# jinseikenai/glomeruli_segmentation

Measured on AMD Instinct MI355X. Metric: patches/sec (1024x512 RGB) ESPNet p=2 q=8 5 classes, HBM-resident, two batches in flight, higher is better.
Workload: dtype f32; 1 GPU; ESPNet p=2 q=8 encoder+decoder, batch=32 synthetic 1024x512 uint8 BGR tiles per GPU, normalise+forward+argmax+counts, inputs resident in HBM, steps rotate through 4 distinct batches, 2 batch(es) in flight (engine lanes, one HIP stream each) for `value`; global_batch=32, weights=espnet_fold1 (tests/golden), parallelism=tile-range per rank x1

## Files before the change

### glomeruli_segmentation_amd/build.py

```python
import os
import subprocess
import sys
import tempfile

PKG = os.path.dirname(os.path.abspath(__file__))
CSRC = os.path.join(PKG, "csrc")
LIB = os.path.join(PKG, "libglomseg.so")
SOURCES = ["espnet.hip", "dec_tail.hip", "crops.hip", "detect_ops.hip", "detector.hip", "wsi_eval.hip", "contours.cpp"]
HEADERS = ["gs_internal.h", "conv_mfma.h", "dec_tail.h", "dec_tail_args.h", "espnet_kernels.h", "crop_sample.h", "crop_plan.h", "host_copy.h", "host_jobs.h", "host_pipe.h",
           os.path.join("..", "..", "include", "glomseg.h")]
FLAGS = ["-O3", "--offload-arch=gfx950", "-std=c++17", "-fPIC", "-Wall", "-Wno-unused-result",
         "-Wno-unused-value"]


def _sources():
    return [s for s in SOURCES if os.path.exists(os.path.join(CSRC, s))]


def _stale(lib):
    if not os.path.exists(lib):
        return True
    t = os.path.getmtime(lib)
    deps = [os.path.join(CSRC, s) for s in _sources() + HEADERS] + [os.path.abspath(__file__)]
    deps += [os.path.join(CSRC, f) for f in os.listdir(CSRC) if f.endswith(".h") or f.endswith(".inc")]
    return any(os.path.getmtime(d) > t for d in deps)


def build_lib(force=False, verbose=False, out=None, extra_flags=()):
    lib = os.path.abspath(out) if out else LIB
    if not (force or _stale(lib)):
        return lib
    hipcc = os.environ.get("HIPCC", "/opt/rocm/bin/hipcc")
    os.makedirs(os.path.dirname(lib), exist_ok=True)
    objdir = CSRC if out is None else tempfile.mkdtemp(prefix="glomseg_obj_")
    objs = []
    procs = []
    for s in _sources():
        o = os.path.join(objdir, s.replace(".hip", ".o").replace(".cpp", ".o"))
        objs.append(o)
        cmd = [hipcc] + FLAGS + list(extra_flags) + (["-x", "hip"] if s.endswith(".cpp") else []) + ["-c", os.path.join(CSRC, s), "-o", o]
        if verbose:
            print(" ".join(cmd))
        procs.append((cmd, subprocess.Popen(cmd)))
    for cmd, p in procs:
        if p.wait() != 0:
            raise RuntimeError("hipcc failed: " + " ".join(cmd))
    cmd = [hipcc, "--offload-arch=gfx950", "-shared", "-fPIC", "-o", lib] + objs + ["-Wl,-rpath,/opt/rocm/lib"]
    if verbose:
        print(" ".join(cmd))
    subprocess.check_call(cmd)
    return lib


if __name__ == "__main__":
    argv = sys.argv[1:]
    extra = []
    if "--" in argv:
        extra = argv[argv.index("--") + 1:]
        argv = argv[:argv.index("--")]
    out = argv[argv.index("--out") + 1] if "--out" in argv else None
    print(build_lib(force="--force" in argv or out is not None, verbose=True, out=out, extra_flags=extra))
```

### glomeruli_segmentation_amd/csrc/conv_mfma.h

```cpp
#pragma once
#include <map>
#include <mutex>
#include <type_traits>

#include "gs_internal.h"

namespace gs {

#ifdef GS_DIAG
constexpr bool kDiag = true;
#else
constexpr bool kDiag = false;
#endif

template <int N, typename F>
__device__ __forceinline__ void static_for(F &&f)
{
    if constexpr (N > 0) {
        static_for<N - 1>(f);
        f(std::integral_constant<int, N - 1>{});
    }
}

typedef float f32x16 __attribute__((ext_vector_type(16)));
typedef float f32x4 __attribute__((ext_vector_type(4)));

template <int MT>
struct Mfma;
template <>
struct Mfma<32> {
    static constexpr int KL = 2, NACC = 16;
    using acc_t = f32x16;
    static __device__ __forceinline__ acc_t run(float a, float b, acc_t c)
    {
        return __builtin_amdgcn_mfma_f32_32x32x2f32(a, b, c, 0, 0, 0);
    }
    static __device__ __forceinline__ int row(int r, int kq) { return (r & 3) + 8 * (r >> 2) + 4 * kq; }
};
template <>
struct Mfma<16> {
    static constexpr int KL = 4, NACC = 4;
    using acc_t = f32x4;
    static __device__ __forceinline__ acc_t run(float a, float b, acc_t c)
    {
        return __builtin_amdgcn_mfma_f32_16x16x4f32(a, b, c, 0, 0, 0);
    }
    static __device__ __forceinline__ int row(int r, int kq) { return kq * 4 + r; }
};

struct ConvArgs {
    const float *in;
    long long in_sn;
    int in_sc, in_pitch, in_off;
    unsigned in_img_bytes;
    const float *wpack;
    int wfloats;
    float *out;
    long long out_sn;
    int out_sc, out_pitch, out_off;
    unsigned out_img_bytes, res_img_bytes;
    const float *res;
    long long res_sn;
    int res_sc, res_pitch, res_off;
    float *out2;
    long long out2_sn;
    int out2_sc, out2_pitch, out2_off, out2_coff;
    unsigned out2_img_bytes;
    float *out3;
    long long out3_sn;
    int out3_sc, out3_pitch, out3_off, nout3;
    unsigned out3_img_bytes;
    int bnl_s0, bnl_s1;
    int stagger;
    int prio_mode;
    unsigned long long *stamp;
    int N, H, W;
    int strips;
    int total_tasks;
    int wu;
};

typedef unsigned u32x3_t __attribute__((ext_vector_type(3)));
typedef unsigned u32x2_t __attribute__((ext_vector_type(2)));
typedef unsigned u32x4_t __attribute__((ext_vector_type(4)));

template <int N, int AUX = 0>
__device__ __forceinline__ void buf_load_vec(const __amdgpu_buffer_rsrc_t &rs, int voff, int soff, float *dst)
{
    if constexpr (N == 1) {
        dst[0] = __builtin_bit_cast(float, __builtin_amdgcn_raw_buffer_load_b32(rs, voff, soff, AUX));
    } else if constexpr (N == 2) {
        const u32x2_t v = __builtin_amdgcn_raw_buffer_load_b64(rs, voff, soff, AUX);
        const unsigned e0 = v[0], e1 = v[1];
        dst[0] = __builtin_bit_cast(float, e0);
        dst[1] = __builtin_bit_cast(float, e1);
    } else {
        static_assert(N == 4 || N == 8, "vector width");
#pragma unroll
        for (int h = 0; h < N / 4; ++h) {
            const u32x4_t v = __builtin_amdgcn_raw_buffer_load_b128(rs, voff + 16 * h, soff, AUX);
            const unsigned e0 = v[0], e1 = v[1], e2 = v[2], e3 = v[3];
            dst[4 * h + 0] = __builtin_bit_cast(float, e0);
            dst[4 * h + 1] = __builtin_bit_cast(float, e1);
            dst[4 * h + 2] = __builtin_bit_cast(float, e2);
            dst[4 * h + 3] = __builtin_bit_cast(float, e3);
        }
    }
}
template <int N, int AUX = 0>
__device__ __forceinline__ void buf_store_vec(const __amdgpu_buffer_rsrc_t &rs, int voff, const float *src)
{
    if constexpr (N == 1) {
        __builtin_amdgcn_raw_buffer_store_b32(__builtin_bit_cast(unsigned, src[0]), rs, voff, 0, AUX);
    } else if constexpr (N == 2) {
        u32x2_t v;
        v[0] = __builtin_bit_cast(unsigned, src[0]);
        v[1] = __builtin_bit_cast(unsigned, src[1]);
        __builtin_amdgcn_raw_buffer_store_b64(v, rs, voff, 0, AUX);
    } else {
#pragma unroll
        for (int h = 0; h < N / 4; ++h) {
            u32x4_t v;
#pragma unroll
            for (int j = 0; j < 4; ++j)
                v[j] = __builtin_bit_cast(unsigned, src[4 * h + j]);
            __builtin_amdgcn_raw_buffer_store_b128(v, rs, voff + 16 * h, 0, AUX);
        }
    }
}

__device__ __forceinline__ float prelu_pin(float alpha)
{
    return alpha <= 1.0f ? __builtin_inff() : -__builtin_inff();
}
__device__ __forceinline__ float prelu_med3(float v, float alpha, float pin)
{
    return __builtin_amdgcn_fmed3f(v, alpha * v, pin);
}

constexpr int F_BNACT = 1;
constexpr int F_RES = 2;
constexpr int F_NOSTORE = 4;
constexpr int F_DUAL = 8;
constexpr int F_S2PAIR = 512;
constexpr int F_VEC = 1024;
constexpr int F_RES_NT = 8192;
constexpr int F_ST_NT = 16384;
constexpr int F_ST2_NT = 32768;
constexpr int F_IN_NT = 65536;
constexpr int F_A_GLOBAL = 131072;
constexpr int F_FUSE1X1 = 262144;
constexpr int F_S2_FLIP = 1048576;
constexpr int F_SKIP_PAD = 4194304;
constexpr int F_BNLOAD = 8388608;
constexpr int F_X_NOLOAD = 16;
constexpr int F_X_NOLDS = 32;
constexpr int F_X_NOEPI = 64;
constexpr int F_X_STAMP2 = 4096;
constexpr int STAMP2_SLOTS = 128;
constexpr int F_X_STAMP = 128;
constexpr int F_X_NOEPIMEM = 2097152;
constexpr int F_X_RESL2 = 33554432;
constexpr int F_X_STL2 = 67108864;
constexpr int F_X_ALL = F_X_NOLOAD | F_X_NOLDS | F_X_NOEPI | F_X_STAMP | F_X_STAMP2 | F_X_NOEPIMEM | F_X_RESL2 | F_X_STL2;

struct ConvImage {
    int nrow, cout, w, bn, tab, total;
};
constexpr ConvImage conv_image(int CINP, int TAPS, int NDIL, int NOUT1, int NOUT, bool bn, bool dual = false, int fuse_nacc = 0)
{
    ConvImage im{};
    im.nrow = NOUT1 > NOUT ? NOUT1 : NOUT;
    im.cout = NOUT1 + (NDIL - 1) * NOUT;
    im.w = NDIL * TAPS * CINP * im.nrow;
    im.bn = (bn ? 3 * im.cout : 0) + (dual ? 3 * im.cout : 0);
    im.tab = NDIL * fuse_nacc * 64;
    im.total = (im.w + im.bn + im.tab + 3) / 4 * 4;
    return im;
}

#ifndef CFG_STAGE_ROT
#define CFG_STAGE_ROT 17
#endif
#ifndef CFG_L3_RING
#define CFG_L3_RING 13
#endif
#ifndef CFG_L2_RING
#define CFG_L2_RING 27
#endif
constexpr int conv_ring_depth(int MT, int TAPS, int NDIL, int P, int G)
{
    return (MT == 32 && TAPS == 9 && NDIL == 5 && (P == 1 || P == 2) && G == 13) ? CFG_L3_RING
           : (MT == 16 && TAPS == 9 && NDIL == 5 && P == 4 && G == 9) ? CFG_L2_RING
                                                                    : G * (TAPS == 9 ? 3 : 1);
}

#define M_KL_OF(MT_) (Mfma<MT_>::KL)
template <int MT, int WAVES, int CINP, int TAPS, int STRIDE, int NDIL, int NOUT1, int NOUT, int P, int G, int FLAGS>
__global__ void __launch_bounds__(WAVES * 64, WAVES >= 8 ? WAVES / 8 : 2) conv_mfma_kernel(const ConvArgs a)
{
    constexpr bool BNACT = FLAGS & F_BNACT, RES = FLAGS & F_RES, STORE1 = !(FLAGS & F_NOSTORE), DUAL = FLAGS & F_DUAL;
    constexpr bool S2P = FLAGS & F_S2PAIR;
    constexpr bool VEC = FLAGS & F_VEC;
    constexpr bool AGL = FLAGS & F_A_GLOBAL, FUSE = FLAGS & F_FUSE1X1;
    constexpr bool S2FLIP = FLAGS & F_S2_FLIP;
    constexpr bool SKIP = FLAGS & F_SKIP_PAD;
    constexpr bool BNL = FLAGS & F_BNLOAD;
    static_assert(!BNL || ((FLAGS & F_S2PAIR) && !(FLAGS & (F_BNACT | F_A_GLOBAL | F_VEC))), "F_BNLOAD is for the plain stride-2 reduce");
    static_assert(!SKIP || (TAPS == 9 && STRIDE == 1 && !(FLAGS & F_S2PAIR) && G * M_KL_OF(MT) == CINP),
                  "F_SKIP_PAD: unit-stride 3x3 with one tap row per chunk");
    static_assert(!S2FLIP || (STRIDE == 2 && TAPS == 9 && NDIL == 1), "F_S2_FLIP is for the stride-2 3x3 reduce");
    static_assert(kDiag || !(FLAGS & F_X_ALL), "timing / stamp variants exist in -DGS_DIAG builds only");
    constexpr int IAUX = (FLAGS & F_IN_NT) ? 2 : 0;
    constexpr int RAUX = (FLAGS & F_RES_NT) ? 2 : 0, SAUX = (FLAGS & F_ST_NT) ? 2 : 0, SAUX2 = (FLAGS & F_ST2_NT) ? 2 : 0;
    static_assert(!VEC || (STRIDE == 1 && (P == 2 || P == 4 || P == 8)), "F_VEC needs unit stride and P in {2,4,8}");
    static_assert(!S2P || (STRIDE == 2 && TAPS == 9 && NDIL == 1), "F_S2PAIR is for the stride-2 3x3 reduce");
    using M = Mfma<MT>;
    constexpr int KL = M::KL;
    constexpr int NSTEP = CINP / KL;
    constexpr int NROW = NOUT1 > NOUT ? NOUT1 : NOUT;
    constexpr int COUT = NOUT1 + (NDIL - 1) * NOUT;
    constexpr int TYN = TAPS == 1 ? 1 : 3;
    constexpr int TXN = TAPS == 9 ? 3 : 1;
    constexpr int XSTEP = P * MT;
    constexpr int RGN = TYN * NSTEP;
    constexpr int D = G * TXN;
    constexpr int R = conv_ring_depth(MT, TAPS, NDIL, P, G);
    constexpr int RA = R;
    static_assert(D % R == 0 && (R == D || !(FLAGS & (F_S2PAIR | F_BNLOAD))), "the ring divides the chunk");
    constexpr int CPD = RGN / G;
    constexpr int NCHUNK = NDIL * CPD;
    static_assert(CINP % KL == 0, "k-steps must tile");
    static_assert(TAPS == 1 || TAPS == 9, "1x1 or 3x3");
    static_assert(RGN % G == 0, "chunk must divide the row groups of one dilation");
    static_assert(NROW <= MT, "one MFMA row block");
    constexpr int KSTR = 4;

    extern __shared__ __attribute__((aligned(16))) float lds[];
    const int tid = threadIdx.x;
    unsigned long long tstamp0 = 0;
    if (FLAGS & (F_X_STAMP | F_X_STAMP2))
        tstamp0 = __builtin_amdgcn_s_memrealtime();
    constexpr int WFL = NDIL * TAPS * CINP * NROW;
    constexpr int LDS_SRC0 = AGL ? WFL : 0;
    static_assert(!AGL || WFL % 4 == 0, "LDS-DMA source must stay 16-byte aligned");
    static_assert(!FUSE || (TAPS == 9 && BNACT), "the fused 1x1 follows a branch kernel's epilogue");
    const float *bnp = lds + (WFL - LDS_SRC0);
    constexpr int BNFL = (BNACT ? 3 * COUT : 0) + (DUAL ? 3 * COUT : 0);
    const float *tab = bnp + BNFL;
    constexpr int BNL_C = CINP + M::KL;
    const float *bnl = lds + (conv_image(CINP, TAPS, NDIL, NOUT1, NOUT, BNACT, DUAL, FUSE ? M::NACC : 0).total - LDS_SRC0);
    const __amdgpu_buffer_rsrc_t rsrc_w =
        __builtin_amdgcn_make_buffer_rsrc(const_cast<float *>(a.wpack), 0, AGL ? WFL * 4 : 0, 0x00020000);

    const int lane = tid & 63;
    const int wid = __builtin_amdgcn_readfirstlane(tid >> 6);
    const int px = lane % MT, kq = lane / MT;
    const int xl = VEC ? px * P : px;
    const int voff = (kq * a.in_sc + xl * STRIDE) * 4;
    const int lbase = kq * NROW + (px < NROW ? px : NROW - 1);
    const int vout = (kq * KSTR * a.out_sc + xl) * 4;
    const int vres = RES ? (kq * KSTR * a.res_sc + xl) * 4 : 0;
    const int vout2 = DUAL ? (kq * KSTR * a.out2_sc + xl) * 4 : 0;
    const int vout3 = FUSE ? (kq * KSTR * a.out3_sc + xl) * 4 : 0;
    const int prio_mode = kDiag ? a.prio_mode : 1;
    const bool second_of_simd = WAVES >= 8 ? wid >= WAVES / 2 : blockIdx.x >= gridDim.x / 2;

    const int NB = gridDim.x;
    const int wu = a.wu;
    int t0, t1, tstride;
    if ((NB & 7) == 0) {
        const int xcd = blockIdx.x & 7, per = NB >> 3;
        const int c0 = (int)((long long)a.total_tasks * xcd / 8), c1 = (int)((long long)a.total_tasks * (xcd + 1) / 8);
        t0 = c0 + (blockIdx.x >> 3) * wu + wid;
        t1 = c1;
        tstride = per * wu;
    } else {
        t0 = blockIdx.x * wu + wid;
        t1 = a.total_tasks;
        tstride = NB * wu;
    }
    if (wid >= wu)
        t0 = t1;
    const long long wg = (long long)blockIdx.x * WAVES + wid;
    const int tasks_per_img = a.H * a.strips;
    bool staged = false;

    float aq[RA], bq[S2P ? 1 : R][P];
    float bl[S2P ? G : 1][P][3];

    for (int task = t0; task < t1 || !staged; task += tstride) {
        const bool idle = task >= t1;
        const int tk = idle ? (a.total_tasks - 1) : task;
        const int n = tk / tasks_per_img;
        const int rem = tk - n * tasks_per_img;
        const int img_stride = tstride / tasks_per_img > 0 ? tstride / tasks_per_img : 1;
        const int yrot = SKIP ? a.H / 2 : 0;
        const int y0r = rem / a.strips;
        const int y = SKIP && ((n / img_stride) & 1) ? (y0r + yrot >= a.H ? y0r + yrot - a.H : y0r + yrot) : y0r;
        const int x0 = (rem - y0r * a.strips) * XSTEP;

        const __amdgpu_buffer_rsrc_t rsrc = __builtin_amdgcn_make_buffer_rsrc(
            const_cast<float *>(a.in + (long long)n * a.in_sn), 0, a.in_img_bytes, 0x00020000);
        const int sbase = (a.in_off + y * STRIDE * a.in_pitch + x0 * STRIDE) * 4;
        const int tn = task + tstride < t1 ? task + tstride : tk;
        const int n_n = tn / tasks_per_img;
        const int rem_n = tn - n_n * tasks_per_img;
        const int y0r_n = rem_n / a.strips;
        const int y_n = SKIP && ((n_n / img_stride) & 1) ? (y0r_n + yrot >= a.H ? y0r_n + yrot - a.H : y0r_n + yrot) : y0r_n;
        const __amdgpu_buffer_rsrc_t rsrc_n = __builtin_amdgcn_make_buffer_rsrc(
            const_cast<float *>(a.in + (long long)n_n * a.in_sn), 0, a.in_img_bytes, 0x00020000);
        const int sbase_n = (a.in_off + y_n * STRIDE * a.in_pitch + (rem_n - y0r_n * a.strips) * XSTEP * STRIDE) * 4;
        const bool flip = S2FLIP && (y & 1), flip_n = S2FLIP && (y_n & 1);
        const __amdgpu_buffer_rsrc_t rout =
            __builtin_amdgcn_make_buffer_rsrc(a.out + (long long)n * a.out_sn, 0, a.out_img_bytes, 0x00020000);
        const int sout = (a.out_off + y * a.out_pitch + x0) * 4;
        const __amdgpu_buffer_rsrc_t rres = __builtin_amdgcn_make_buffer_rsrc(
            const_cast<float *>(RES ? a.res + (long long)n * a.res_sn : a.in), 0, RES ? a.res_img_bytes : 0u, 0x00020000);
        const int sres = RES ? (a.res_off + y * a.res_pitch + x0) * 4 : 0;
        const __amdgpu_buffer_rsrc_t rout2 = __builtin_amdgcn_make_buffer_rsrc(
            DUAL ? a.out2 + (long long)n * a.out2_sn : a.out, 0, DUAL ? a.out2_img_bytes : 0u, 0x00020000);
        const int sout2 = DUAL ? (a.out2_off + y * a.out2_pitch + x0) * 4 : 0;
        const __amdgpu_buffer_rsrc_t rout3 = __builtin_amdgcn_make_buffer_rsrc(
            FUSE ? a.out3 + (long long)n * a.out3_sn : a.out, 0, FUSE ? a.out3_img_bytes : 0u, 0x00020000);
        const int sout3 = FUSE ? (a.out3_off + y * a.out3_pitch + x0) * 4 : 0;

        typename M::acc_t acc[P];
        typename M::acc_t acc2[FUSE ? P : 1];
        auto chunk_live = [&](int yy, int c) {
            const int di = c / CPD, ty = c - di * CPD;
            return ty == 1 || (ty == 0 ? yy >= (1 << di) : yy + (1 << di) < a.H);
        };
        const int c_first = SKIP && !chunk_live(y, 0) ? 1 : 0;
        const int c_first_n = SKIP && !chunk_live(y_n, 0) ? 1 : 0;

        constexpr int OOB = 0x7ffffff0;
        int vo[P], vr[P], vo2[P], vo3[P];
#pragma unroll
        for (int p = 0; p < P; ++p) {
            const bool xok = x0 + (VEC ? xl : p * MT + px) < a.W;
            vo[p] = xok ? vout + (VEC ? 0 : p * MT * 4) : OOB;
            vr[p] = xok ? vres + (VEC ? 0 : p * MT * 4) : OOB;
            vo2[p] = xok ? vout2 + (VEC ? 0 : p * MT * 4) : OOB;
            vo3[p] = xok ? vout3 + (VEC ? 0 : p * MT * 4) : OOB;
        }
        constexpr int RR = RES ? M::NACC : 1;
        float resv[RR][P];
        auto load_res = [&](int di, int r) {
            if (!RES)
                return;
            if (FLAGS & F_X_NOEPIMEM) {
#pragma unroll
                for (int p = 0; p < P; ++p)
                    resv[r % RR][p] = __builtin_bit_cast(float, di + r + p);
                return;
            }
            const int nout = di == 0 ? NOUT1 : NOUT;
            const int cb = di == 0 ? 0 : NOUT1 + (di - 1) * NOUT;
            const int ch0 = M::row(r, 0);
            const bool live = ch0 + kq * KSTR < nout;
            const int sr = (cb + ch0) * a.res_sc * 4 + sres;
            if (VEC) {
                if (FLAGS & F_X_RESL2)
                    buf_load_vec<P, RAUX>(rres, live ? ((int)(wg & 255) * 8192 + ((vr[0] + sr) & 0x1ff0)) : OOB, 0, resv[r % RR]);
                else
                    buf_load_vec<P, RAUX>(rres, live ? vr[0] : OOB, sr, resv[r % RR]);
                return;
            }
#pragma unroll
            for (int p = 0; p < P; ++p)
                resv[r % RR][p] = __builtin_bit_cast(
                    float, __builtin_amdgcn_raw_buffer_load_b32(rres, live ? vr[p] : OOB, sr, RAUX));
        };
        auto prefetch_res = [&](int di) {
#pragma unroll
            for (int r = 0; r < RR; ++r)
                load_res(di, r);
        };

        auto decode_rg = [&](int cw, int g, int &ty0, int &sidx) {
            if constexpr (G % NSTEP == 0) {
                ty0 = cw * (G / NSTEP) + g / NSTEP;
                sidx = g % NSTEP;
            } else if constexpr (NSTEP % G == 0) {
                constexpr int CPR = NSTEP / G;
                ty0 = cw / CPR;
                sidx = (cw - ty0 * CPR) * G + g;
            } else {
                const int rg = cw * G + g;
                ty0 = rg / NSTEP;
                sidx = rg - ty0 * NSTEP;
            }
        };
        auto fetch_b = [&](const __amdgpu_buffer_rsrc_t &rs, int sb, int c, int g, int tx, bool fl) {
            const int di = c / CPD;
            int ty0, sidx;
            decode_rg(c - di * CPD, g, ty0, sidx);
            const int ty = S2FLIP && fl ? TYN - 1 - ty0 : ty0;
            const int toff = TAPS == 9 ? ((ty - 1) * a.in_pitch + (tx - 1)) << di : 0;
            const int soff = sb + (toff + sidx * KL * a.in_sc) * 4;
            if ((FLAGS & F_X_NOLOAD) && staged)
                return;
            if (VEC) {
                buf_load_vec<P, IAUX>(rs, voff, soff, bq[S2P ? 0 : (g * TXN + tx) % R]);
                return;
            }
#pragma unroll
            for (int p = 0; p < P; ++p)
                bq[(g * TXN + tx) % R][p] = __builtin_bit_cast(
                    float, __builtin_amdgcn_raw_buffer_load_b32(rs, voff + p * MT * STRIDE * 4, soff, IAUX));
        };
        auto fetch_pair = [&](const __amdgpu_buffer_rsrc_t &rs, int sb, int c, int g, bool fl) {
            if ((FLAGS & F_X_NOLOAD) && staged)
                return;
            int ty0, sidx;
            decode_rg(c, g, ty0, sidx);
            const int ty = S2FLIP && fl ? TYN - 1 - ty0 : ty0;
            const int soff = sb + ((ty - 1) * a.in_pitch - 1 + sidx * KL * a.in_sc) * 4;
#pragma unroll
            for (int p = 0; p < P; ++p) {
                const u32x3_t v = __builtin_amdgcn_raw_buffer_load_b96(rs, voff + p * MT * STRIDE * 4, soff, IAUX);
                const unsigned e0 = v[0], e1 = v[1], e2 = v[2];
                bl[g][p][0] = __builtin_bit_cast(float, e0);
                bl[g][p][1] = __builtin_bit_cast(float, e1);
                bl[g][p][2] = __builtin_bit_cast(float, e2);
            }
        };
        auto fetch_a = [&](int c, int g, int tx, bool fl) {
            const int di = c / CPD;
            int ty0, sidx;
            decode_rg(c - di * CPD, g, ty0, sidx);
            const int ty = S2FLIP && fl ? TYN - 1 - ty0 : ty0;
            const int tap = TAPS == 9 ? ty * 3 + tx : 0;
            if ((FLAGS & F_X_NOLDS) && staged)
                return;
            if (AGL)
                aq[(g * TXN + tx) % R] = __builtin_bit_cast(
                    float, __builtin_amdgcn_raw_buffer_load_b32(rsrc_w, lbase * 4, (((di * TAPS + tap) * CINP + sidx * KL) * NROW) * 4, 0));
            else
                aq[(g * TXN + tx) % R] = lds[((di * TAPS + tap) * CINP + sidx * KL) * NROW + lbase];
        };

        auto bnl_fetch = [&](int cc, int gg, int yy, bool ff, float &sc2, float &sh2, float &al2, bool &raw) {
            int ty0c, sidxc;
            decode_rg(cc, gg, ty0c, sidxc);
            const int tyc = S2FLIP && ff ? TYN - 1 - ty0c : ty0c;
            raw = sidxc >= a.bnl_s0 && sidxc < a.bnl_s1;
            const bool padrow = yy * STRIDE + tyc - 1 < 0 && raw;
            const int ch = (padrow ? NSTEP : sidxc) * KL + kq;
            sc2 = bnl[ch];
            sh2 = bnl[BNL_C + ch];
            al2 = bnl[2 * BNL_C + ch];
        };
        float tsc = 1.0f, tsh = 0.0f, tal = 1.0f, tpin = 0.0f;
        float nsc = 1.0f, nsh = 0.0f, nal = 1.0f;
        bool traw = false, nraw = false;
        float bt[BNL ? 2 : 1][P][3];
        static_assert(!BNL || G % 2 == 0, "F_BNLOAD: the two-group operand buffer alternates by row-group parity");
        auto bnl_apply = [&](float &dst, float v, float sc2, float sh2, float al2, float pin2, bool zero) {
            v = v * sc2 + sh2;
            v = prelu_med3(v, al2, pin2);
            dst = zero ? 0.0f : v;
        };

        if (task == t0) {
#pragma unroll
            for (int g = 0; g < G; ++g) {
                if (S2P) {
                    fetch_pair(rsrc, sbase, 0, g, flip);
                    continue;
                }
#pragma unroll
                for (int tx = 0; tx < TXN; ++tx)
                    if (g * TXN + tx < R)
                        fetch_b(rsrc, sbase, c_first, g, tx, flip);
            }
        }
        if (!staged) {
            const int pieces = (a.wfloats - LDS_SRC0 + 255) / 256;
            if ((FLAGS & F_X_STAMP2) && lane == 0)
                a.stamp[wg * STAMP2_SLOTS + STAMP2_SLOTS - 2] = __builtin_amdgcn_s_memrealtime();
            const int rot = (int)((blockIdx.x * (unsigned)CFG_STAGE_ROT) % (unsigned)(pieces > 0 ? pieces : 1));
            for (int j0 = wid; j0 < pieces; j0 += WAVES) {
                const int j = j0 + rot < pieces ? j0 + rot : j0 + rot - pieces;
                __builtin_amdgcn_global_load_lds(
                    (const __attribute__((address_space(1))) void *)(a.wpack + LDS_SRC0 + j * 256 + lane * 4),
                    (__attribute__((address_space(3))) void *)(lds + j * 256), 16, 0, 0);
            }
            if ((FLAGS & F_X_STAMP2) && lane == 0)
                a.stamp[wg * STAMP2_SLOTS + STAMP2_SLOTS - 1] = __builtin_amdgcn_s_memrealtime();
            __syncthreads();
            staged = true;
        }
        if (idle)
            break;
        if ((FLAGS & F_X_STAMP) && lane == 0 && task == t0) {
            a.stamp[wg * 8 + 0] = tstamp0;
            a.stamp[wg * 8 + 1] = __builtin_amdgcn_s_memrealtime();
        }
        if ((FLAGS & F_X_STAMP2) && lane == 0 && task == t0) {
            a.stamp[wg * STAMP2_SLOTS + 0] = tstamp0;
            a.stamp[wg * STAMP2_SLOTS + 1] = __builtin_amdgcn_s_memrealtime();
        }
        const int ti_ = (FLAGS & F_X_STAMP2) ? (task - t0) / tstride : 0;
        const bool stamp2 = (FLAGS & F_X_STAMP2) && lane == 0 && 2 + (ti_ + 1) * 2 * NCHUNK <= STAMP2_SLOTS;
        const long long sbase2 = wg * STAMP2_SLOTS + 2 + ti_ * 2 * NCHUNK;
        if (kDiag && a.stagger > 0 && task == t0) {
            const int ph = second_of_simd ? 1 : 0;
            for (int z = 0; z < a.stagger * ph; ++z)
                __builtin_amdgcn_s_sleep(16);
        }
        if (task == t0) {
#pragma unroll
            for (int g = 0; g < G; ++g)
#pragma unroll
                for (int tx = 0; tx < TXN; ++tx)
                    if (g * TXN + tx < R)
                        fetch_a(c_first, g, tx, flip);
        }

        if (BNL) {
            bnl_fetch(c_first, 0, y, flip, tsc, tsh, tal, traw);
            bnl_fetch(c_first, 1, y, flip, nsc, nsh, nal, nraw);
            tpin = prelu_pin(tal);
#pragma unroll
            for (int p = 0; p < P; ++p)
#pragma unroll
                for (int t = 0; t < 3; ++t)
                    bnl_apply(bt[0][p][t], bl[0][p][t], tsc, tsh, tal, tpin, t == 0 && p == 0 && x0 == 0 && px == 0);
        }
        if (FUSE) {
#pragma unroll
            for (int p = 0; p < P; ++p)
                acc2[p] = (typename M::acc_t)(0.0f);
        }
        if (prio_mode == 1) {
            if ((((task - t0) / tstride) + (second_of_simd ? 1 : 0)) & 1)
                __builtin_amdgcn_s_setprio(1);
            else
                __builtin_amdgcn_s_setprio(0);
        } else if (prio_mode == 3 && task == t0) {
            if (second_of_simd)
                __builtin_amdgcn_s_setprio(1);
        }

        struct EpiParams {
            float scale = 1.0f, shift = 0.0f, alpha = 1.0f, scale2 = 1.0f, shift2 = 0.0f, alpha2 = 1.0f, a2 = 0.0f;
        };
        auto epi_params = [&](int di, auto r_) __attribute__((always_inline)) {
            constexpr int r = decltype(r_)::value;
            const int nout = di == 0 ? NOUT1 : NOUT;
            const int cb = di == 0 ? 0 : NOUT1 + (di - 1) * NOUT;
            const int ch0 = M::row(r, 0);
            const bool live = ch0 + kq * KSTR < nout;
            EpiParams q;
            q.a2 = (FUSE && BNACT) ? tab[(di * M::NACC + r) * 64 + lane] : 0.0f;
            if (BNACT) {
                const float *bp = bnp + (live ? cb + ch0 + kq * KSTR : 0);
                q.scale = bp[0];
                q.shift = bp[COUT];
                q.alpha = bp[2 * COUT];
                if (DUAL) {
                    q.scale2 = bp[3 * COUT];
                    q.shift2 = bp[4 * COUT];
                    q.alpha2 = bp[5 * COUT];
                }
            }
            return q;
        };
        auto epi_reg = [&](int di, auto r_) __attribute__((always_inline)) {
            constexpr int r = decltype(r_)::value;
            const int nout = di == 0 ? NOUT1 : NOUT;
            const int cb = di == 0 ? 0 : NOUT1 + (di - 1) * NOUT;
            const int ch0 = M::row(r, 0);
            const bool live = ch0 + kq * KSTR < nout;
            const EpiParams q = epi_params(di, r_);
            const float a2 = q.a2;
            const int so = (cb + ch0) * a.out_sc * 4 + sout;
            const int so2 = DUAL ? (a.out2_coff + cb + ch0) * a.out2_sc * 4 + sout2 : 0;
            const float scale = q.scale, shift = q.shift, alpha = q.alpha, scale2 = q.scale2, shift2 = q.shift2, alpha2 = q.alpha2;
            float o1[P], o2[P];
            const float pin = prelu_pin(alpha), pin2 = prelu_pin(alpha2);
#pragma unroll
            for (int p = 0; p < P; ++p) {
                float v = acc[p][r];
                if (RES)
                    v += resv[r % RR][p];
                if (BNACT) {
                    v = v * scale + shift;
                    v = prelu_med3(v, alpha, pin);
                }
                o1[p] = v;
                if (!VEC && STORE1)
                    __builtin_amdgcn_raw_buffer_store_b32(__builtin_bit_cast(unsigned, v), rout, live ? vo[p] : OOB, so, SAUX);
                if (DUAL) {
                    float v2 = v * scale2 + shift2;
                    v2 = prelu_med3(v2, alpha2, pin2);
                    o2[p] = v2;
                    if (!VEC)
                        __builtin_amdgcn_raw_buffer_store_b32(__builtin_bit_cast(unsigned, v2), rout2,
                                                              live ? vo2[p] : OOB, so2, SAUX2);
                }
            }
            if (VEC && STORE1 && !(FLAGS & F_X_NOEPIMEM))
                buf_store_vec<P, SAUX>(rout, live ? ((FLAGS & F_X_STL2) ? ((int)(wg & 255) * 8192 + ((vo[0] + so) & 0x1ff0)) : vo[0] + so) : OOB, o1);
            if (VEC && DUAL)
                buf_store_vec<P, SAUX2>(rout2, live ? vo2[0] + so2 : OOB, o2);
            if (FUSE && ch0 < nout) {
#pragma unroll
                for (int p = 0; p < P; ++p)
                    acc2[p] = M::run(a2, o1[p], acc2[p]);
            }
        };

        for (int c = 0; c < NCHUNK; ++c) {
            if (NDIL > 1 && c % CPD == 0 && prio_mode == 0) {
                if (((c / CPD) + (second_of_simd ? 1 : 0)) & 1)
                    __builtin_amdgcn_s_setprio(1);
                else
                    __builtin_amdgcn_s_setprio(0);
            }
            if (RES && c % CPD == 0)
                prefetch_res(c / CPD);
            if (c % CPD == 0 && c < 2 * CPD) {
#pragma unroll
                for (int p = 0; p < P; ++p)
                    acc[p] = (typename M::acc_t)(0.0f);
            }
            int nxl = c + 1;
            if (SKIP)
                while (nxl < NCHUNK && !chunk_live(y, nxl))
                    ++nxl;
            const bool last = nxl >= NCHUNK;
            const int nx = last ? c_first_n : nxl;
            const __amdgpu_buffer_rsrc_t rs = last ? rsrc_n : rsrc;
            const int sb = last ? sbase_n : sbase;
            const bool fl = last ? flip_n : flip;
            auto refill = [&](int u) __attribute__((always_inline)) {
                const int v = u + R;
                if (v < D && R < D) {
                    fetch_b(rsrc, sbase, c, v / TXN, v % TXN, flip);
                    fetch_a(c, v / TXN, v % TXN, flip);
                } else {
                    const int gn = (v - D) / TXN, txn = (v - D) % TXN;
                    if (!S2P)
                        fetch_b(rs, sb, nx, gn, txn, fl);
                    else if (txn == 2)
                        fetch_pair(rs, sb, nx, gn, fl);
                    fetch_a(nx, gn, txn, fl);
                }
            };
            if (!SKIP || chunk_live(y, c)) {
#pragma unroll
            for (int g = 0; g < G; ++g)
#pragma unroll
                for (int tx = 0; tx < TXN; ++tx) {
                    const int u = g * TXN + tx;
                    const bool ahead = BNL && (g + 1 < G || !last);
                    if (BNL && tx == 0) {
                        tsc = nsc;
                        tsh = nsh;
                        tal = nal;
                        traw = nraw;
                        tpin = prelu_pin(tal);
                        if (g + 2 < G)
                            bnl_fetch(c, g + 2, y, flip, nsc, nsh, nal, nraw);
                        else if (!last)
                            bnl_fetch(nx, g + 2 - G, y, flip, nsc, nsh, nal, nraw);
                    }
#pragma unroll
                    for (int p = 0; p < P; ++p) {
                        acc[p] = M::run(aq[u % RA], BNL ? bt[BNL ? g & 1 : 0][p][S2P ? tx : 0]
                                                       : S2P ? bl[S2P ? g : 0][p][S2P ? tx : 0] : bq[S2P ? 0 : u % R][p], acc[p]);
                        if (ahead) {
                            const int e = tx * P + p;
                            if (e < 3 * P)
                                bnl_apply(bt[BNL ? (g + 1) & 1 : 0][e / 3][e % 3], bl[S2P ? (g + 1) % G : 0][e / 3][e % 3], tsc, tsh, tal, tpin,
                                          e == 0 && x0 == 0 && px == 0);
                        }
                    }
                    refill(u);
                    __builtin_amdgcn_sched_barrier(0);
                }
            }
            if (stamp2)
                a.stamp[sbase2 + 2 * c] = __builtin_amdgcn_s_memrealtime();
            if ((c + 1) % CPD != 0)
                continue;
            if (FLAGS & F_X_NOEPI) {
                float keep = 0.0f;
#pragma unroll
                for (int p = 0; p < P; ++p)
#pragma unroll
                    for (int r = 0; r < M::NACC; ++r)
                        keep += acc[p][r];
                if (keep == 123.456f)
                    __builtin_amdgcn_raw_buffer_store_b32(__builtin_bit_cast(unsigned, keep), rout, vout, sout, 0);
                continue;
            }
            const int di = c / CPD;
            static_for<M::NACC>([&](auto r_) { epi_reg(di, r_); });
            if (FUSE && di + 1 == NDIL) {
#pragma unroll
                for (int r = 0; r < M::NACC; ++r) {
                    const int ch0 = M::row(r, 0);
                    if (ch0 >= a.nout3)
                        continue;
                    const bool live3 = ch0 + kq * KSTR < a.nout3;
                    const int so3 = ch0 * a.out3_sc * 4 + sout3;
                    float o3[P];
#pragma unroll
                    for (int p = 0; p < P; ++p) {
                        o3[p] = acc2[p][r];
                        if (!VEC)
                            __builtin_amdgcn_raw_buffer_store_b32(__builtin_bit_cast(unsigned, o3[p]), rout3, live3 ? vo3[p] : OOB, so3, 0);
                    }
                    if (VEC)
                        buf_store_vec<P, 0>(rout3, live3 ? vo3[0] + so3 : OOB, o3);
                }
            }
            if ((FLAGS & F_X_STAMP) && lane == 0 && task == t0)
                a.stamp[wg * 8 + 2 + di] = __builtin_amdgcn_s_memrealtime();
            if (stamp2)
                a.stamp[sbase2 + 2 * c + 1] = __builtin_amdgcn_s_memrealtime();
        }
    }
}

constexpr int conv_wfloats(int CINP, int TAPS, int NDIL, int NOUT1, int NOUT, bool bn, bool dual = false, int fuse_nacc = 0)
{
    return conv_image(CINP, TAPS, NDIL, NOUT1, NOUT, bn, dual, fuse_nacc).total;
}

struct LaunchInfo {
    bool attr_done = false;
    int per_cu = 0;
};

template <int MT, int WAVES, int CINP, int TAPS, int STRIDE, int NDIL, int NOUT1, int NOUT, int P, int G, int FLAGS>
gs_status launch_conv_mfma(ConvArgs a, int num_cus, hipStream_t stream)
{
    auto kern = conv_mfma_kernel<MT, WAVES, CINP, TAPS, STRIDE, NDIL, NOUT1, NOUT, P, G, FLAGS>;
    constexpr ConvImage im = conv_image(CINP, TAPS, NDIL, NOUT1, NOUT, FLAGS & F_BNACT, FLAGS & F_DUAL,
                                        (FLAGS & F_FUSE1X1) ? Mfma<MT>::NACC : 0);
    a.strips = cdiv(a.W, P * MT);
    a.total_tasks = a.N * a.H * a.strips;
    a.prio_mode = 1;
#ifdef GS_DIAG
    if (const char *e = std::getenv("GS_PRIO"))
        a.prio_mode = std::atoi(e);
    if (const char *e = std::getenv("GS_STAGGER"))
        a.stagger = std::atoi(e);
#endif
    constexpr int EXTRA = (FLAGS & F_BNLOAD) ? 3 * (CINP + Mfma<MT>::KL) : 0;
    a.wfloats = im.total + EXTRA;
    const int lds_floats = im.total + EXTRA - ((FLAGS & F_A_GLOBAL) ? im.w : 0);
    const size_t lds_bytes = (size_t)((lds_floats + 255) / 256 * 256) * sizeof(float);
    static std::mutex mu;
    static std::map<int, LaunchInfo> by_device;
    int dev = 0;
    GS_HIP(hipGetDevice(&dev));
    int per_cu;
    {
        std::lock_guard<std::mutex> lock(mu);
        LaunchInfo &li = by_device[dev];
        if (!li.attr_done) {
            GS_HIP(hipFuncSetAttribute(reinterpret_cast<const void *>(kern), hipFuncAttributeMaxDynamicSharedMemorySize,
                                       (int)lds_bytes));
            li.attr_done = true;
        }
        if (li.per_cu == 0) {
            int nb = 0;
            GS_HIP(hipOccupancyMaxActiveBlocksPerMultiprocessor(&nb, reinterpret_cast<const void *>(kern), WAVES * 64, lds_bytes));
            li.per_cu = nb < 1 ? 1 : nb;
        }
        per_cu = li.per_cu;
    }
    int grid = num_cus * per_cu;
    if (grid >= 8) grid = grid / 8 * 8;
    a.wu = WAVES;
    if ((long long)a.total_tasks < (long long)grid * WAVES) {
        a.wu = cdiv(a.total_tasks, grid);
        if (a.wu < 1) a.wu = 1;
        int g = cdiv(a.total_tasks, a.wu);
        if (g >= 8) g = (g + 7) / 8 * 8;
        grid = g < grid ? g : grid;
    }
    if (grid < 1) grid = 1;
    hipLaunchKernelGGL(kern, dim3(grid), dim3(WAVES * 64), lds_bytes, stream, a);
    GS_HIP(hipGetLastError());
    return GS_OK;
}

}
```

Measured before the change: 11550 patches/s.

## Hoist weight staging and first-task prefetch out of conv task loop; precompute task geometry

Moves the LDS weight staging (global_load_lds) and the first task's input/weight fetch ahead of the main loop, so the kernel issues one barrier before any work instead of doing it inside the first loop iteration. Task decode now uses host-precomputed geometry and multiply-shift division in place of integer divides, guarded by an exactness check. The XCD task split is derived from precomputed quotient and remainder. This trims per-task scalar work and lets the weight DMA overlap with the first input fetch, at the cost of more kernel arguments and a more complex prologue.

```diff
diff --git a/glomeruli_segmentation_amd/build.py b/glomeruli_segmentation_amd/build.py
--- a/glomeruli_segmentation_amd/build.py
+++ b/glomeruli_segmentation_amd/build.py
@@ -7,7 +7,7 @@
 CSRC = os.path.join(PKG, "csrc")
 LIB = os.path.join(PKG, "libglomseg.so")
 SOURCES = ["espnet.hip", "dec_tail.hip", "crops.hip", "detect_ops.hip", "detector.hip", "wsi_eval.hip", "contours.cpp"]
-HEADERS = ["gs_internal.h", "conv_mfma.h", "dec_tail.h", "dec_tail_args.h", "espnet_kernels.h", "crop_sample.h", "crop_plan.h", "host_copy.h", "host_jobs.h", "host_pipe.h",
+HEADERS = ["gs_internal.h", "conv_mfma.h", "conv_task_geom.h", "dec_tail.h", "dec_tail_args.h", "espnet_kernels.h", "crop_sample.h", "crop_plan.h", "host_copy.h", "host_jobs.h", "host_pipe.h",
            os.path.join("..", "..", "include", "glomseg.h")]
 FLAGS = ["-O3", "--offload-arch=gfx950", "-std=c++17", "-fPIC", "-Wall", "-Wno-unused-result",
          "-Wno-unused-value"]
diff --git a/glomeruli_segmentation_amd/csrc/conv_mfma.h b/glomeruli_segmentation_amd/csrc/conv_mfma.h
--- a/glomeruli_segmentation_amd/csrc/conv_mfma.h
+++ b/glomeruli_segmentation_amd/csrc/conv_mfma.h
@@ -3,6 +3,7 @@
 #include <mutex>
 #include <type_traits>
 
+#include "conv_task_geom.h"
 #include "gs_internal.h"
 
 namespace gs {
@@ -54,7 +55,6 @@
     int in_sc, in_pitch, in_off;
     unsigned in_img_bytes;
     const float *wpack;
-    int wfloats;
     float *out;
     long long out_sn;
     int out_sc, out_pitch, out_off;
@@ -75,9 +75,12 @@
     int prio_mode;
     unsigned long long *stamp;
     int N, H, W;
+    int wu;
     int strips;
-    int total_tasks;
-    int wu;
+    int total_tasks, tasks_per_img, tasks_q8, tasks_r8, tstride, img_stride;
+    unsigned mul_img, mul_strips, mul_img_stride;
+    int sh_img, sh_strips, sh_img_stride;
+    int fast_div;
 };
 
 typedef unsigned u32x3_t __attribute__((ext_vector_type(3)));
@@ -255,6 +258,24 @@
 
     const int lane = tid & 63;
     const int wid = __builtin_amdgcn_readfirstlane(tid >> 6);
+
+    constexpr int EXTRA_FL = BNL ? 3 * BNL_C : 0;
+    constexpr int PIECES = (conv_image(CINP, TAPS, NDIL, NOUT1, NOUT, BNACT, DUAL, FUSE ? M::NACC : 0).total + EXTRA_FL - LDS_SRC0 + 255) / 256;
+    const long long wg = (long long)blockIdx.x * WAVES + wid;
+    if ((FLAGS & F_X_STAMP2) && lane == 0)
+        a.stamp[wg * STAMP2_SLOTS + STAMP2_SLOTS - 2] = __builtin_amdgcn_s_memrealtime();
+    if constexpr (PIECES > 0) {
+        const int rot = (int)((blockIdx.x * (unsigned)CFG_STAGE_ROT) % (unsigned)PIECES);
+        for (int j0 = wid; j0 < PIECES; j0 += WAVES) {
+            const int j = j0 + rot < PIECES ? j0 + rot : j0 + rot - PIECES;
+            __builtin_amdgcn_global_load_lds(
+                (const __attribute__((address_space(1))) void *)(a.wpack + LDS_SRC0 + j * 256 + lane * 4),
+                (__attribute__((address_space(3))) void *)(lds + j * 256), 16, 0, 0);
+        }
+    }
+    if ((FLAGS & F_X_STAMP2) && lane == 0)
+        a.stamp[wg * STAMP2_SLOTS + STAMP2_SLOTS - 1] = __builtin_amdgcn_s_memrealtime();
+    __builtin_amdgcn_sched_barrier(0);
     const int px = lane % MT, kq = lane / MT;
     const int xl = VEC ? px * P : px;
     const int voff = (kq * a.in_sc + xl * STRIDE) * 4;
@@ -268,49 +289,161 @@
 
     const int NB = gridDim.x;
     const int wu = a.wu;
-    int t0, t1, tstride;
+    const int tstride = a.tstride;
+    int t0, t1;
     if ((NB & 7) == 0) {
-        const int xcd = blockIdx.x & 7, per = NB >> 3;
-        const int c0 = (int)((long long)a.total_tasks * xcd / 8), c1 = (int)((long long)a.total_tasks * (xcd + 1) / 8);
-        t0 = c0 + (blockIdx.x >> 3) * wu + wid;
-        t1 = c1;
-        tstride = per * wu;
+        const int xcd = blockIdx.x & 7;
+        t0 = xcd_first_task(a.tasks_q8, a.tasks_r8, xcd) + (blockIdx.x >> 3) * wu + wid;
+        t1 = xcd_first_task(a.tasks_q8, a.tasks_r8, xcd + 1);
     } else {
         t0 = blockIdx.x * wu + wid;
         t1 = a.total_tasks;
-        tstride = NB * wu;
-    }
-    if (wid >= wu)
-        t0 = t1;
-    const long long wg = (long long)blockIdx.x * WAVES + wid;
-    const int tasks_per_img = a.H * a.strips;
-    bool staged = false;
+    }
+    const bool has_task = wid < wu && t0 < t1;
+    auto quot = [&](int x, int d, unsigned mul, int shift) {
+        return a.fast_div ? (int)(((unsigned long long)(unsigned)x * mul) >> shift) : x / d;
+    };
+    auto decode_task = [&](int tk, int &n, int &y, int &x0) {
+        n = quot(tk, a.tasks_per_img, a.mul_img, a.sh_img);
+        const int rem = tk - n * a.tasks_per_img;
+        const int y0r = quot(rem, a.strips, a.mul_strips, a.sh_strips);
+        const int yrot = y0r + a.H / 2 >= a.H ? y0r + a.H / 2 - a.H : y0r + a.H / 2;
+        y = SKIP && (quot(n, a.img_stride, a.mul_img_stride, a.sh_img_stride) & 1) ? yrot : y0r;
+        x0 = (rem - y0r * a.strips) * XSTEP;
+    };
+    auto in_rsrc = [&](int n) {
+        return __builtin_amdgcn_make_buffer_rsrc(const_cast<float *>(a.in + (long long)n * a.in_sn), 0, a.in_img_bytes, 0x00020000);
+    };
+    auto in_base = [&](int y, int x0) { return (a.in_off + y * STRIDE * a.in_pitch + x0 * STRIDE) * 4; };
+    auto chunk_live = [&](int yy, int c) {
+        const int di = c / CPD, ty = c - di * CPD;
+        return ty == 1 || (ty == 0 ? yy >= (1 << di) : yy + (1 << di) < a.H);
+    };
 
     float aq[RA], bq[S2P ? 1 : R][P];
     float bl[S2P ? G : 1][P][3];
-
-    for (int task = t0; task < t1 || !staged; task += tstride) {
-        const bool idle = task >= t1;
-        const int tk = idle ? (a.total_tasks - 1) : task;
-        const int n = tk / tasks_per_img;
-        const int rem = tk - n * tasks_per_img;
-        const int img_stride = tstride / tasks_per_img > 0 ? tstride / tasks_per_img : 1;
-        const int yrot = SKIP ? a.H / 2 : 0;
-        const int y0r = rem / a.strips;
-        const int y = SKIP && ((n / img_stride) & 1) ? (y0r + yrot >= a.H ? y0r + yrot - a.H : y0r + yrot) : y0r;
-        const int x0 = (rem - y0r * a.strips) * XSTEP;
-
-        const __amdgpu_buffer_rsrc_t rsrc = __builtin_amdgcn_make_buffer_rsrc(
-            const_cast<float *>(a.in + (long long)n * a.in_sn), 0, a.in_img_bytes, 0x00020000);
-        const int sbase = (a.in_off + y * STRIDE * a.in_pitch + x0 * STRIDE) * 4;
-        const int tn = task + tstride < t1 ? task + tstride : tk;
-        const int n_n = tn / tasks_per_img;
-        const int rem_n = tn - n_n * tasks_per_img;
-        const int y0r_n = rem_n / a.strips;
-        const int y_n = SKIP && ((n_n / img_stride) & 1) ? (y0r_n + yrot >= a.H ? y0r_n + yrot - a.H : y0r_n + yrot) : y0r_n;
-        const __amdgpu_buffer_rsrc_t rsrc_n = __builtin_amdgcn_make_buffer_rsrc(
-            const_cast<float *>(a.in + (long long)n_n * a.in_sn), 0, a.in_img_bytes, 0x00020000);
-        const int sbase_n = (a.in_off + y_n * STRIDE * a.in_pitch + (rem_n - y0r_n * a.strips) * XSTEP * STRIDE) * 4;
+    bool warm = false;
+
+    auto decode_rg = [&](int cw, int g, int &ty0, int &sidx) {
+        if constexpr (G % NSTEP == 0) {
+            ty0 = cw * (G / NSTEP) + g / NSTEP;
+            sidx = g % NSTEP;
+        } else if constexpr (NSTEP % G == 0) {
+            constexpr int CPR = NSTEP / G;
+            ty0 = cw / CPR;
+            sidx = (cw - ty0 * CPR) * G + g;
+        } else {
+            const int rg = cw * G + g;
+            ty0 = rg / NSTEP;
+            sidx = rg - ty0 * NSTEP;
+        }
+    };
+    auto fetch_b = [&](const __amdgpu_buffer_rsrc_t &rs, int sb, int c, int g, int tx, bool fl) {
+        const int di = c / CPD;
+        int ty0, sidx;
+        decode_rg(c - di * CPD, g, ty0, sidx);
+        const int ty = S2FLIP && fl ? TYN - 1 - ty0 : ty0;
+        const int toff = TAPS == 9 ? ((ty - 1) * a.in_pitch + (tx - 1)) << di : 0;
+        const int soff = sb + (toff + sidx * KL * a.in_sc) * 4;
+        if ((FLAGS & F_X_NOLOAD) && warm)
+            return;
+        if (VEC) {
+            buf_load_vec<P, IAUX>(rs, voff, soff, bq[S2P ? 0 : (g * TXN + tx) % R]);
+            return;
+        }
+#pragma unroll
+        for (int p = 0; p < P; ++p)
+            bq[(g * TXN + tx) % R][p] = __builtin_bit_cast(
+                float, __builtin_amdgcn_raw_buffer_load_b32(rs, voff + p * MT * STRIDE * 4, soff, IAUX));
+    };
+    auto fetch_pair = [&](const __amdgpu_buffer_rsrc_t &rs, int sb, int c, int g, bool fl) {
+        if ((FLAGS & F_X_NOLOAD) && warm)
+            return;
+        int ty0, sidx;
+        decode_rg(c, g, ty0, sidx);
+        const int ty = S2FLIP && fl ? TYN - 1 - ty0 : ty0;
+        const int soff = sb + ((ty - 1) * a.in_pitch - 1 + sidx * KL * a.in_sc) * 4;
+#pragma unroll
+        for (int p = 0; p < P; ++p) {
+            const u32x3_t v = __builtin_amdgcn_raw_buffer_load_b96(rs, voff + p * MT * STRIDE * 4, soff, IAUX);
+            const unsigned e0 = v[0], e1 = v[1], e2 = v[2];
+            bl[g][p][0] = __builtin_bit_cast(float, e0);
+            bl[g][p][1] = __builtin_bit_cast(float, e1);
+            bl[g][p][2] = __builtin_bit_cast(float, e2);
+        }
+    };
+    auto fetch_a = [&](int c, int g, int tx, bool fl) {
+        const int di = c / CPD;
+        int ty0, sidx;
+        decode_rg(c - di * CPD, g, ty0, sidx);
+        const int ty = S2FLIP && fl ? TYN - 1 - ty0 : ty0;
+        const int tap = TAPS == 9 ? ty * 3 + tx : 0;
+        if ((FLAGS & F_X_NOLDS) && warm)
+            return;
+        if (AGL)
+            aq[(g * TXN + tx) % R] = __builtin_bit_cast(
+                float, __builtin_amdgcn_raw_buffer_load_b32(rsrc_w, lbase * 4, (((di * TAPS + tap) * CINP + sidx * KL) * NROW) * 4, 0));
+        else
+            aq[(g * TXN + tx) % R] = lds[((di * TAPS + tap) * CINP + sidx * KL) * NROW + lbase];
+    };
+
+    int n_nx = 0, y_nx = 0, x0_nx = 0;
+    if (has_task) {
+        decode_task(t0, n_nx, y_nx, x0_nx);
+        const __amdgpu_buffer_rsrc_t rsrc_f = in_rsrc(n_nx);
+        const int sbase_f = in_base(y_nx, x0_nx);
+        const bool flip_f = S2FLIP && (y_nx & 1);
+        const int c_first_f = SKIP && !chunk_live(y_nx, 0) ? 1 : 0;
+#pragma unroll
+        for (int g = 0; g < G; ++g) {
+            if (S2P) {
+                fetch_pair(rsrc_f, sbase_f, 0, g, flip_f);
+                continue;
+            }
+#pragma unroll
+            for (int tx = 0; tx < TXN; ++tx)
+                if (g * TXN + tx < R)
+                    fetch_b(rsrc_f, sbase_f, c_first_f, g, tx, flip_f);
+        }
+    }
+    __syncthreads();
+    if (!has_task)
+        return;
+    if ((FLAGS & F_X_STAMP) && lane == 0) {
+        a.stamp[wg * 8 + 0] = tstamp0;
+        a.stamp[wg * 8 + 1] = __builtin_amdgcn_s_memrealtime();
+    }
+    if ((FLAGS & F_X_STAMP2) && lane == 0) {
+        a.stamp[wg * STAMP2_SLOTS + 0] = tstamp0;
+        a.stamp[wg * STAMP2_SLOTS + 1] = __builtin_amdgcn_s_memrealtime();
+    }
+    if (kDiag && a.stagger > 0) {
+        const int ph = second_of_simd ? 1 : 0;
+        for (int z = 0; z < a.stagger * ph; ++z)
+            __builtin_amdgcn_s_sleep(16);
+    }
+    {
+        const bool flip_f = S2FLIP && (y_nx & 1);
+        const int c_first_f = SKIP && !chunk_live(y_nx, 0) ? 1 : 0;
+#pragma unroll
+        for (int g = 0; g < G; ++g)
+#pragma unroll
+            for (int tx = 0; tx < TXN; ++tx)
+                if (g * TXN + tx < R)
+                    fetch_a(c_first_f, g, tx, flip_f);
+    }
+    warm = true;
+
+    int ti = 0;
+    for (int task = t0; task < t1; task += tstride, ++ti) {
+        const int n = n_nx, y = y_nx, x0 = x0_nx;
+        const __amdgpu_buffer_rsrc_t rsrc = in_rsrc(n);
+        const int sbase = in_base(y, x0);
+        if (task + tstride < t1)
+            decode_task(task + tstride, n_nx, y_nx, x0_nx);
+        const int y_n = y_nx;
+        const __amdgpu_buffer_rsrc_t rsrc_n = in_rsrc(n_nx);
+        const int sbase_n = in_base(y_nx, x0_nx);
         const bool flip = S2FLIP && (y & 1), flip_n = S2FLIP && (y_n & 1);
         const __amdgpu_buffer_rsrc_t rout =
             __builtin_amdgcn_make_buffer_rsrc(a.out + (long long)n * a.out_sn, 0, a.out_img_bytes, 0x00020000);
@@ -327,10 +460,6 @@
 
         typename M::acc_t acc[P];
         typename M::acc_t acc2[FUSE ? P : 1];
-        auto chunk_live = [&](int yy, int c) {
-            const int di = c / CPD, ty = c - di * CPD;
-            return ty == 1 || (ty == 0 ? yy >= (1 << di) : yy + (1 << di) < a.H);
-        };
         const int c_first = SKIP && !chunk_live(y, 0) ? 1 : 0;
         const int c_first_n = SKIP && !chunk_live(y_n, 0) ? 1 : 0;
 
@@ -376,69 +505,6 @@
 #pragma unroll
             for (int r = 0; r < RR; ++r)
                 load_res(di, r);
-        };
-
-        auto decode_rg = [&](int cw, int g, int &ty0, int &sidx) {
-            if constexpr (G % NSTEP == 0) {
-                ty0 = cw * (G / NSTEP) + g / NSTEP;
-                sidx = g % NSTEP;
-            } else if constexpr (NSTEP % G == 0) {
-                constexpr int CPR = NSTEP / G;
-                ty0 = cw / CPR;
-                sidx = (cw - ty0 * CPR) * G + g;
-            } else {
-                const int rg = cw * G + g;
-                ty0 = rg / NSTEP;
-                sidx = rg - ty0 * NSTEP;
-            }
-        };
-        auto fetch_b = [&](const __amdgpu_buffer_rsrc_t &rs, int sb, int c, int g, int tx, bool fl) {
-            const int di = c / CPD;
-            int ty0, sidx;
-            decode_rg(c - di * CPD, g, ty0, sidx);
-            const int ty = S2FLIP && fl ? TYN - 1 - ty0 : ty0;
-            const int toff = TAPS == 9 ? ((ty - 1) * a.in_pitch + (tx - 1)) << di : 0;
-            const int soff = sb + (toff + sidx * KL * a.in_sc) * 4;
-            if ((FLAGS & F_X_NOLOAD) && staged)
-                return;
-            if (VEC) {
-                buf_load_vec<P, IAUX>(rs, voff, soff, bq[S2P ? 0 : (g * TXN + tx) % R]);
-                return;
-            }
-#pragma unroll
-            for (int p = 0; p < P; ++p)
-                bq[(g * TXN + tx) % R][p] = __builtin_bit_cast(
-                    float, __builtin_amdgcn_raw_buffer_load_b32(rs, voff + p * MT * STRIDE * 4, soff, IAUX));
-        };
-        auto fetch_pair = [&](const __amdgpu_buffer_rsrc_t &rs, int sb, int c, int g, bool fl) {
-            if ((FLAGS & F_X_NOLOAD) && staged)
-                return;
-            int ty0, sidx;
-            decode_rg(c, g, ty0, sidx);
-            const int ty = S2FLIP && fl ? TYN - 1 - ty0 : ty0;
-            const int soff = sb + ((ty - 1) * a.in_pitch - 1 + sidx * KL * a.in_sc) * 4;
-#pragma unroll
-            for (int p = 0; p < P; ++p) {
-                const u32x3_t v = __builtin_amdgcn_raw_buffer_load_b96(rs, voff + p * MT * STRIDE * 4, soff, IAUX);
-                const unsigned e0 = v[0], e1 = v[1], e2 = v[2];
-                bl[g][p][0] = __builtin_bit_cast(float, e0);
-                bl[g][p][1] = __builtin_bit_cast(float, e1);
-                bl[g][p][2] = __builtin_bit_cast(float, e2);
-            }
-        };
-        auto fetch_a = [&](int c, int g, int tx, bool fl) {
-            const int di = c / CPD;
-            int ty0, sidx;
-            decode_rg(c - di * CPD, g, ty0, sidx);
-            const int ty = S2FLIP && fl ? TYN - 1 - ty0 : ty0;
-            const int tap = TAPS == 9 ? ty * 3 + tx : 0;
-            if ((FLAGS & F_X_NOLDS) && staged)
-                return;
-            if (AGL)
-                aq[(g * TXN + tx) % R] = __builtin_bit_cast(
-                    float, __builtin_amdgcn_raw_buffer_load_b32(rsrc_w, lbase * 4, (((di * TAPS + tap) * CINP + sidx * KL) * NROW) * 4, 0));
-            else
-                aq[(g * TXN + tx) % R] = lds[((di * TAPS + tap) * CINP + sidx * KL) * NROW + lbase];
         };
 
         auto bnl_fetch = [&](int cc, int gg, int yy, bool ff, float &sc2, float &sh2, float &al2, bool &raw) {
@@ -463,61 +529,9 @@
             dst = zero ? 0.0f : v;
         };
 
-        if (task == t0) {
-#pragma unroll
-            for (int g = 0; g < G; ++g) {
-                if (S2P) {
-                    fetch_pair(rsrc, sbase, 0, g, flip);
-                    continue;
-                }
-#pragma unroll
-                for (int tx = 0; tx < TXN; ++tx)
-                    if (g * TXN + tx < R)
-                        fetch_b(rsrc, sbase, c_first, g, tx, flip);
-            }
-        }
-        if (!staged) {
-            const int pieces = (a.wfloats - LDS_SRC0 + 255) / 256;
-            if ((FLAGS & F_X_STAMP2) && lane == 0)
-                a.stamp[wg * STAMP2_SLOTS + STAMP2_SLOTS - 2] = __builtin_amdgcn_s_memrealtime();
-            const int rot = (int)((blockIdx.x * (unsigned)CFG_STAGE_ROT) % (unsigned)(pieces > 0 ? pieces : 1));
-            for (int j0 = wid; j0 < pieces; j0 += WAVES) {
-                const int j = j0 + rot < pieces ? j0 + rot : j0 + rot - pieces;
-                __builtin_amdgcn_global_load_lds(
-                    (const __attribute__((address_space(1))) void *)(a.wpack + LDS_SRC0 + j * 256 + lane * 4),
-                    (__attribute__((address_space(3))) void *)(lds + j * 256), 16, 0, 0);
-            }
-            if ((FLAGS & F_X_STAMP2) && lane == 0)
-                a.stamp[wg * STAMP2_SLOTS + STAMP2_SLOTS - 1] = __builtin_amdgcn_s_memrealtime();
-            __syncthreads();
-            staged = true;
-        }
-        if (idle)
-            break;
-        if ((FLAGS & F_X_STAMP) && lane == 0 && task == t0) {
-            a.stamp[wg * 8 + 0] = tstamp0;
-            a.stamp[wg * 8 + 1] = __builtin_amdgcn_s_memrealtime();
-        }
-        if ((FLAGS & F_X_STAMP2) && lane == 0 && task == t0) {
-            a.stamp[wg * STAMP2_SLOTS + 0] = tstamp0;
-            a.stamp[wg * STAMP2_SLOTS + 1] = __builtin_amdgcn_s_memrealtime();
-        }
-        const int ti_ = (FLAGS & F_X_STAMP2) ? (task - t0) / tstride : 0;
+        const int ti_ = (FLAGS & F_X_STAMP2) ? ti : 0;
         const bool stamp2 = (FLAGS & F_X_STAMP2) && lane == 0 && 2 + (ti_ + 1) * 2 * NCHUNK <= STAMP2_SLOTS;
         const long long sbase2 = wg * STAMP2_SLOTS + 2 + ti_ * 2 * NCHUNK;
-        if (kDiag && a.stagger > 0 && task == t0) {
-            const int ph = second_of_simd ? 1 : 0;
-            for (int z = 0; z < a.stagger * ph; ++z)
-                __builtin_amdgcn_s_sleep(16);
-        }
-        if (task == t0) {
-#pragma unroll
-            for (int g = 0; g < G; ++g)
-#pragma unroll
-                for (int tx = 0; tx < TXN; ++tx)
-                    if (g * TXN + tx < R)
-                        fetch_a(c_first, g, tx, flip);
-        }
 
         if (BNL) {
             bnl_fetch(c_first, 0, y, flip, tsc, tsh, tal, traw);
@@ -535,11 +549,11 @@
                 acc2[p] = (typename M::acc_t)(0.0f);
         }
         if (prio_mode == 1) {
-            if ((((task - t0) / tstride) + (second_of_simd ? 1 : 0)) & 1)
+            if ((ti + (second_of_simd ? 1 : 0)) & 1)
                 __builtin_amdgcn_s_setprio(1);
             else
                 __builtin_amdgcn_s_setprio(0);
-        } else if (prio_mode == 3 && task == t0) {
+        } else if (prio_mode == 3 && ti == 0) {
             if (second_of_simd)
                 __builtin_amdgcn_s_setprio(1);
         }
@@ -719,7 +733,7 @@
                         buf_store_vec<P, 0>(rout3, live3 ? vo3[0] + so3 : OOB, o3);
                 }
             }
-            if ((FLAGS & F_X_STAMP) && lane == 0 && task == t0)
+            if ((FLAGS & F_X_STAMP) && lane == 0 && ti == 0)
                 a.stamp[wg * 8 + 2 + di] = __builtin_amdgcn_s_memrealtime();
             if (stamp2)
                 a.stamp[sbase2 + 2 * c + 1] = __builtin_amdgcn_s_memrealtime();
@@ -753,7 +767,6 @@
         a.stagger = std::atoi(e);
 #endif
     constexpr int EXTRA = (FLAGS & F_BNLOAD) ? 3 * (CINP + Mfma<MT>::KL) : 0;
-    a.wfloats = im.total + EXTRA;
     const int lds_floats = im.total + EXTRA - ((FLAGS & F_A_GLOBAL) ? im.w : 0);
     const size_t lds_bytes = (size_t)((lds_floats + 255) / 256 * 256) * sizeof(float);
     static std::mutex mu;
@@ -787,6 +800,19 @@
         grid = g < grid ? g : grid;
     }
     if (grid < 1) grid = 1;
+    const ConvTaskGeom tg = conv_task_geom(a.N, a.H, a.W, P * MT, grid, a.wu);
+    a.tasks_per_img = tg.tasks_per_img;
+    a.tasks_q8 = tg.tasks_q8;
+    a.tasks_r8 = tg.tasks_r8;
+    a.tstride = tg.tstride;
+    a.img_stride = tg.img_stride;
+    a.mul_img = tg.by_img.mul;
+    a.sh_img = tg.by_img.shift;
+    a.mul_strips = tg.by_strips.mul;
+    a.sh_strips = tg.by_strips.shift;
+    a.mul_img_stride = tg.by_img_stride.mul;
+    a.sh_img_stride = tg.by_img_stride.shift;
+    a.fast_div = tg.fast_div;
     hipLaunchKernelGGL(kern, dim3(grid), dim3(WAVES * 64), lds_bytes, stream, a);
     GS_HIP(hipGetLastError());
     return GS_OK;
diff --git a/glomeruli_segmentation_amd/csrc/conv_task_geom.h b/glomeruli_segmentation_amd/csrc/conv_task_geom.h
--- /dev/null
+++ b/glomeruli_segmentation_amd/csrc/conv_task_geom.h
@@ -0,0 +1,71 @@
+#pragma once
+
+namespace gs {
+
+struct MulShift {
+    unsigned mul = 0;
+    int shift = 0;
+};
+constexpr MulShift mulshift_for(unsigned d)
+{
+    int l = 0;
+    while ((1ull << l) < d)
+        ++l;
+    MulShift ms;
+    ms.shift = 31 + l;
+    ms.mul = (unsigned)(((1ull << ms.shift) + d - 1) / d);
+    return ms;
+}
+constexpr unsigned mulshift_div(unsigned x, MulShift ms) { return (unsigned)(((unsigned long long)x * ms.mul) >> ms.shift); }
+
+constexpr bool mulshift_exact_below(unsigned d, unsigned limit)
+{
+    if (d == 0 || d >= (1u << 31))
+        return false;
+    if (limit == 0)
+        return true;
+    const MulShift ms = mulshift_for(d);
+    const unsigned long long two = 1ull << ms.shift, e = (unsigned long long)ms.mul * d - two;
+    const unsigned xm = limit - 1, qm = xm / d, rm = xm - qm * d;
+    if (qm * e + (unsigned long long)rm * ms.mul >= two)
+        return false;
+    if (rm != d - 1 && qm > 0 && (qm - 1) * e + (unsigned long long)(d - 1) * ms.mul >= two)
+        return false;
+    return true;
+}
+
+struct ConvTaskGeom {
+    int strips = 0;
+    int tasks_per_img = 0;
+    int total_tasks = 0;
+    int tasks_q8 = 0, tasks_r8 = 0;
+    int tstride = 0;
+    int img_stride = 1;
+    MulShift by_img, by_strips, by_img_stride;
+    int fast_div = 0;
+};
+
+constexpr int xcd_first_task(int q8, int r8, int x) { return q8 * x + ((r8 * x) >> 3); }
+
+constexpr ConvTaskGeom conv_task_geom(int N, int H, int W, int xstep, int grid, int wu)
+{
+    ConvTaskGeom g;
+    g.strips = (W + xstep - 1) / xstep;
+    g.tasks_per_img = H * g.strips;
+    g.total_tasks = N * g.tasks_per_img;
+    g.tasks_q8 = g.total_tasks >> 3;
+    g.tasks_r8 = g.total_tasks & 7;
+    g.tstride = ((grid & 7) == 0 ? grid >> 3 : grid) * wu;
+    g.img_stride = g.tasks_per_img > 0 && g.tstride / g.tasks_per_img > 0 ? g.tstride / g.tasks_per_img : 1;
+    if (g.total_tasks > 0) {
+        g.by_img = mulshift_for((unsigned)g.tasks_per_img);
+        g.by_strips = mulshift_for((unsigned)g.strips);
+        g.by_img_stride = mulshift_for((unsigned)g.img_stride);
+        g.fast_div = mulshift_exact_below((unsigned)g.tasks_per_img, (unsigned)g.total_tasks) &&
+                     mulshift_exact_below((unsigned)g.strips, (unsigned)g.tasks_per_img) &&
+                     mulshift_exact_below((unsigned)g.img_stride, (unsigned)N);
+    }
+    return g;
+}
+
+}
```

After: 11610 patches/s, median of 6. About the same (+0.4%).
